# cuMF/cumf_als

Hardware: AMD Instinct MI355X
Metric: ratings/sec per ALS half-iteration (Netflix f=100); RMSE vs reference (higher is better)
Workload: dtype f32 (bf16x3-split products on the bf16 matrix pipe, fp32 accumulate); 1 GPU; netflix-shape synthetic ratings 17770x480189, nnz=99072112, f=100, lambda=0.048, solver=lu, X_BATCH=1 THETA_BATCH=1, fused Gram+solve; step=update-X + update-Theta (two half-iterations)

## Files before the change

### cumf_als_amd/als.py

```python
from __future__ import annotations

import ctypes as C

import numpy as np

from . import lib as _libmod

SOLVER_CG, SOLVER_LU = 0, 1
CUMF_ERR_FAST_RANGE = 10001


def _solver_id(solver) -> int:
    if solver in (SOLVER_CG, "cg", "CG"):
        return SOLVER_CG
    if solver in (SOLVER_LU, "lu", "LU"):
        return SOLVER_LU
    raise ValueError(f"unknown solver {solver!r}")


def _hostptr(a: np.ndarray, dtype) -> C.c_void_p:
    if a.dtype != dtype or not a.flags["C_CONTIGUOUS"]:
        raise TypeError(f"expected C-contiguous {np.dtype(dtype).name} array")
    return a.ctypes.data_as(C.c_void_p)

# ... 255 lines not shown

def lu_solve(A, b, x=None):
    import torch

    lib = _libmod.load()
    f = b.shape[-1]
    batch = b.numel() // f
    if x is None:
        x = torch.empty_like(b)
    _libmod.check(lib.cumf_lu_solve_batched(_dp(A, torch.float32), _dp(b, torch.float32), _dp(x, torch.float32),
                                            batch, f, _stream()), "cumf_lu_solve_batched")
    return x


def pack_upper(full, packed=None):
    import torch

    lib = _libmod.load()
    batch, f = full.shape[0], full.shape[-1]
    if packed is None:
        packed = torch.empty((batch, f * (f + 1) // 2), dtype=torch.float32, device=full.device)
    _libmod.check(lib.cumf_pack_upper(_dp(full, torch.float32), _dp(packed, torch.float32), batch, f, _stream()),
                  "cumf_pack_upper")
    return packed


def unpack_upper(packed, full):
    import torch

    lib = _libmod.load()
    batch, f = full.shape[0], full.shape[-1]
    _libmod.check(lib.cumf_unpack_upper(_dp(packed, torch.float32), _dp(full, torch.float32), batch, f, _stream()),
                  "cumf_unpack_upper")
    return full


def sse(val, row, col, thetaT, XT, count: int | None = None, surpass_nan: bool = False, out=None):
    import torch

    lib = _libmod.load()
    f = thetaT.shape[-1]
    if count is None:
        count = val.numel()
    if out is None:
        out = torch.zeros(1, dtype=torch.float64, device=val.device)
    _libmod.check(lib.cumf_sse(_dp(val, torch.float32), _dp(row, torch.int32), _dp(col, torch.int32),
                               _dp(thetaT, torch.float32), _dp(XT, torch.float32), int(count), f,
                               int(bool(surpass_nan)), _dp(out, torch.float64), _stream()), "cumf_sse")
    return out


GRAM_AUTO, GRAM_EXACT, GRAM_FAST = 0, 1, 2


def set_gram_mode(mode) -> None:
    m = {"auto": GRAM_AUTO, "split": GRAM_AUTO, "exact": GRAM_EXACT, "fast": GRAM_FAST}.get(mode, mode)
    _libmod.check(_libmod.load().cumf_set_gram_mode(int(m)), "cumf_set_gram_mode")


def get_gram_mode() -> str:
    return {GRAM_EXACT: "exact", GRAM_FAST: "fast"}.get(_libmod.load().cumf_get_gram_mode(), "auto")


PRESPLIT_AUTO, PRESPLIT_OFF, PRESPLIT_ON, PRESPLIT_VERIFY = -1, 0, 1, 2


def set_presplit(mode) -> None:
    m = {"auto": PRESPLIT_AUTO, "off": PRESPLIT_OFF, "on": PRESPLIT_ON, "verify": PRESPLIT_VERIFY}.get(mode, mode)
    _libmod.check(_libmod.load().cumf_set_presplit(int(m)), "cumf_set_presplit")


def get_presplit() -> str:
    return {PRESPLIT_OFF: "off", PRESPLIT_ON: "on", PRESPLIT_VERIFY: "verify"}.get(_libmod.load().cumf_get_presplit(), "auto")


def presplit_table(table: "torch.Tensor") -> "torch.Tensor":
    import torch

    lib = _libmod.load()
    rows, f = int(table.shape[0]), int(table.shape[1])
    pitch = int(lib.cumf_presplit_pitch(f))
    if pitch == 0:
        raise ValueError(f"no pre-split kernels for f = {f}")
    out = torch.empty((rows, pitch), dtype=torch.uint8, device=table.device)
    _libmod.check(lib.cumf_presplit_table(_dp(table, torch.float32), out.data_ptr(), rows, f, _stream()), "cumf_presplit_table")
    return out


def gram_fast_status() -> int:
    import ctypes as C

    flags = C.c_int(0)
    _libmod.check(_libmod.load().cumf_gram_fast_status(C.byref(flags)), "cumf_gram_fast_status")
    return int(flags.value)


def check_gram_fast() -> None:
    if _libmod.load().cumf_get_gram_mode() != GRAM_FAST:
        return
    flags = gram_fast_status()
    if flags:
        what = " and ".join(w for b, w in ((1, "a factor"), (2, "a rating")) if flags & b)
        raise RuntimeError(f"gram mode 'fast': {what} beyond the f16 range of the pre-split operands "
                           "(|value| >= 15.99): use the default gram mode")


def set_debug_switches(switches: int) -> None:
    lib = _libmod.load()
    if not hasattr(lib, "cumf_set_debug_switches"):
        raise RuntimeError("ablation switches exist only in libALS_ablate.so (load it through CUMF_ALS_LIB)")
    _libmod.check(lib.cumf_set_debug_switches(int(switches)), "cumf_set_debug_switches")


def debug_cg_histogram(f: int):
    lib = _libmod.load()
    if not hasattr(lib, "cumf_debug_cg_histogram"):
        raise RuntimeError("the CG histogram exists only in libALS_ablate.so (load it through CUMF_ALS_LIB)")
    out = (C.c_ulonglong * 16)()
    _libmod.check(lib.cumf_debug_cg_histogram(int(f), out), "cumf_debug_cg_histogram")
    return [int(v) for v in out]


def last_kernel_name() -> str:
    buf = C.create_string_buffer(256)
    _libmod.check(_libmod.load().cumf_last_kernel_name(buf, 256), "cumf_last_kernel_name")
    return buf.value.decode()


def last_tile_batches():
    info = (C.c_long * 2)()
    _libmod.check(_libmod.load().cumf_last_tile_batches(info), "cumf_last_tile_batches")
    return int(info[0]), int(info[1])


def set_kernel_timing(enable: bool) -> None:
    _libmod.check(_libmod.load().cumf_set_kernel_timing(int(bool(enable))), "cumf_set_kernel_timing")


def last_kernel_ms():
    a, b = C.c_float(), C.c_float()
    _libmod.check(_libmod.load().cumf_last_kernel_ms(C.byref(a), C.byref(b)), "cumf_last_kernel_ms")
    return a.value, b.value


def kernel_ms_since_reset():
    a, b, n = C.c_float(), C.c_float(), C.c_int()
    _libmod.check(_libmod.load().cumf_kernel_ms_since_reset(C.byref(a), C.byref(b), C.byref(n)),
                  "cumf_kernel_ms_since_reset")
    return a.value, b.value, n.value


def release_scratch() -> None:
    _libmod.check(_libmod.load().cumf_release_scratch(), "cumf_release_scratch")



NNLS_MAX_F = 128


def nnls_available(f: int) -> bool:
    return bool(_libmod.load().cumf_nnls_available(int(f)))


def _check_nonneg_f(f: int) -> None:
    if not (8 <= int(f) <= NNLS_MAX_F and int(f) % 2 == 0):
        raise ValueError(f"non-negative ALS takes even 8 <= f <= {NNLS_MAX_F} (got f = {f})")

# ... 719 lines not shown
```

### cumf_als_amd/csrc/als_capi.cpp

```cpp
#include <hip/hip_runtime.h>

#include <cxxabi.h>

#include <algorithm>
#include <cmath>
#include <cstdint>
#include <cstdio>
#include <cstdlib>
#include <cstring>
#include <vector>

#include "als_internal.h"
#include "cg.h"
#include "cumf_als_capi.h"

using namespace cumf;

namespace {

#if CUMF_ABLATE
int g_debug_switches = -1;
int debug_switches() {
  if (g_debug_switches < 0) g_debug_switches = getenv("CUMF_ALS_DBG") ? atoi(getenv("CUMF_ALS_DBG")) : 0;
  return g_debug_switches;
}
#endif

KernelArgs base_args(const cumf_plan_t* p, const int* colidx, const float* val, const float* gather, int f,
                     float lambda) {
  KernelArgs a{};
  a.item_row = p->d_item_row;
  a.item_begin = p->d_item_begin;
  a.item_len = p->d_item_len;
  a.item_slot = p->d_item_slot;
  a.item_rowlen = p->d_item_rowlen;
  a.mrow_row = p->d_mrow_row;
  a.mrow_slot0 = p->d_mrow_slot0;
  a.mrow_nslots = p->d_mrow_nslots;
  a.mrow_rowlen = p->d_mrow_rowlen;
  a.part = p->d_part;
  a.colidx = colidx;
  a.val = val;
  a.gather = gather;
  a.gather_f32 = gather;
  a.row_begin = p->row_begin;
  a.f = f;
  a.lambda = lambda;
#if CUMF_ABLATE
  a.dbg = debug_switches();
#endif
  return a;
}

int fast_words(const cumf_plan_t* p, const float* gather, int f, hipStream_t stream, KernelArgs* a) {
  if (p->gather_rows <= 0) {
    fprintf(stderr, "cumf_als_update_fused: gram mode \"fast\" needs the row count of the gather table "
                    "(cumf_plan_set_gather_rows)\n");
    return (int)hipErrorInvalidValue;
  }
  const size_t n = (size_t)p->gather_rows * f;
  void* words = nullptr;
  int rc = scratch_get(stream, kScratchWords, n * sizeof(unsigned), &words);
  if (rc) return rc;
  int* flag = nullptr;
  rc = fast_flag_get(&flag);
  if (rc) return rc;
  CUMF_HIP_CHECK(launch_presplit(gather, static_cast<unsigned*>(words), n, flag, stream));
  a->gather = reinterpret_cast<const float*>(words);
  a->fast_flag = flag;
  return 0;
}

int pre_words(const cumf_plan_t* p, const float* gather, int f, hipStream_t stream, KernelArgs* a) {
  void* planes = nullptr;
  const int rc = scratch_get(stream, kScratchPlanes, (size_t)p->gather_rows * presplit_pitch(f), &planes);
  if (rc) return rc;
  CUMF_HIP_CHECK(launch_presplit3(gather, planes, p->gather_rows, f, stream));
  a->gather = reinterpret_cast<const float*>(planes);
  a->pre_pitch = presplit_pitch(f);
  return 0;
}

thread_local int g_last_error = 0;

}


extern "C" int cumf_last_error(void) {
  const int e = g_last_error;
  g_last_error = 0;
  return e;
}
void cumf::set_last_error(int code) { g_last_error = code; }

extern "C" int cumf_last_kernel_name(char* buf, int cap) {
  if (!buf || cap <= 0) return (int)hipErrorInvalidValue;
  buf[0] = 0;
  const void* fn = last_item_kernel();
  if (!fn) return 0;
  const char* mangled = hipKernelNameRefByPtr(fn, nullptr);
  if (!mangled) return 0;
  int status = 0;
  char* dem = abi::__cxa_demangle(mangled, nullptr, nullptr, &status);
  const char* name = (status == 0 && dem) ? dem : mangled;
  size_t len = strlen(name);
  int depth = 0;
  for (size_t i = 0; name[i]; ++i) {
    if (name[i] == '<') ++depth;
    if (name[i] == '>') --depth;
    if (name[i] == '(' && depth == 0) {
      len = i;
      break;
    }
  }
  if (strncmp(name, "void ", 5) == 0) {
    name += 5;
    len -= 5;
  }
  if (len >= (size_t)cap) len = (size_t)cap - 1;
  memcpy(buf, name, len);
  buf[len] = 0;
  free(dem);
  return 0;
}

extern "C" int cumf_fused_available(int f, int solver) {
  const int mode = solver == CUMF_SOLVER_LU ? kModeLU : kModeCG;
  if (f <= 0 || (f % 2) != 0 || (solver != CUMF_SOLVER_CG && solver != CUMF_SOLVER_LU)) return 0;
  return route_for(f, mode, PlanFacts{}, switches()).path != kPathNone;
}

namespace {
int update_fused_impl(const cumf_plan_t* p, const int* colidx, const float* val, const float* gather, float* update, int f,
                      float lambda, int solver, int cg_iters, double* sse_bins, void* stream) {
  if (!p || f != p->f) {
    fprintf(stderr, "cumf_als_update_fused: plan/f mismatch\n");
    return (int)hipErrorInvalidValue;
  }
  if (!cumf_fused_available(f, solver)) {
    fprintf(stderr, "cumf_als_update_fused: f = %d with this solver needs the materialising path "
                    "(cumf_get_hermitian + cumf_*_solve_batched): the fused LU serves even f <= %d, the fused CG "
                    "too except in gram mode exact (the full system in LDS, f <= %d)\n", f, kMaxF, kVecLd);
    return (int)hipErrorInvalidValue;
  }
  ScratchLease lease;
  KernelArgs a = base_args(p, colidx, val, gather, f, lambda);
  a.update = update;
  a.cg_iters = cg_iters;
  a.sse_bins = sse_bins;
  const int mode = (solver == CUMF_SOLVER_LU) ? kModeLU : kModeCG;
  const Route r = route_for(f, mode, plan_facts(p), switches());
  PlanLists lists{};
  int rc = plan_lists(p, &lists, static_cast<hipStream_t>(stream), r.whole == kSolveTileBuffer);
  if (!rc && r.table == kTableF16Words) rc = fast_words(p, gather, f, static_cast<hipStream_t>(stream), &a);
  if (!rc && r.table == kTablePlanes) rc = pre_words(p, gather, f, static_cast<hipStream_t>(stream), &a);
  if (rc) return rc;
  CUMF_HIP_CHECK(launch_half_iteration(a, mode, r, lists, static_cast<hipStream_t>(stream)));
  return 0;
}
}

extern "C" int cumf_als_update_fused(const cumf_plan_t* p, const int* colidx, const float* val, const float* gather,
// ... 272 lines not shown
```

### cumf_als_amd/csrc/als_dual.hip

```cpp
#include <hip/hip_runtime.h>

#include "als_device.h"
#include "als_internal.h"
#include "als_lu_blocked.h"
#include "als_wave_gram.h"
#include "als_wave_solve.h"

namespace cumf {

namespace {

constexpr int kDualFB = 6;
constexpr int kDualPlane = 32 * kDualFB;
constexpr int kDualChunks = kDualFB / 2;
constexpr int kDualStrip = 96 * kDualFB;
constexpr int kDualWaves = 3;
constexpr int kDualPass = 40;

template <class T>
__device__ __forceinline__ __attribute__((address_space(1))) const T* as_global(const void* p) {
  return reinterpret_cast<__attribute__((address_space(1))) const T*>(reinterpret_cast<unsigned long long>(p));
}

template <int NBD>
__host__ __device__ constexpr int dual_lds_floats() {
  return wave_lu_lds_floats<NBD>(16 * NBD - 1) + 16 * NBD + 16;
}

template <int NBD, int KC>
__device__ __forceinline__ void dual_load_chunk(const char* const (&ptr)[NBD], u32x4 (&op)[NBD][3]) {
  static_for<NBD>([&](auto ic) {
    constexpr int I = decltype(ic)::value;
    static_for<3>([&](auto pc) {
      constexpr int p = decltype(pc)::value;
      op[I][p] = *as_global<u32x4>(ptr[I] + kDualPlane * p + 64 * KC);
    });
  });
}
template <int NBD>
__device__ __forceinline__ void dual_products(const u32x4 (&op)[NBD][3], f32x4 (&acc)[NBD * (NBD + 1) / 2]) {
  static_for<6>([&](auto prc) {
    constexpr int PROD = decltype(prc)::value;
    constexpr int pa = PROD == 0 ? 2 : (PROD == 2 || PROD == 3) ? 1 : 0;
    constexpr int pb = PROD == 1 ? 2 : (PROD == 2 || PROD == 4) ? 1 : 0;
    static_for<NBD*(NBD + 1) / 2>([&](auto tc) {
      constexpr int t = decltype(tc)::value;
      constexpr int I = tile_I<NBD>(t), J = tile_J<NBD>(t);
      acc[t] = mfma_bf16(op[I][pa], op[J][pb], acc[t]);
    });
  });
}

template <int NBD>
__global__ __launch_bounds__(64, kDualWaves) void als_dual_kernel(const KernelArgs a) {
  extern __shared__ __attribute__((aligned(16))) float smem[];
  constexpr int NT = NBD * (NBD + 1) / 2;
  constexpr int kMaxN = 16 * NBD - 1;
  const int lane = threadIdx.x;
  const int item = blockIdx.x;
  const int row = a.item_row[item];
  const long long begin = a.item_begin[item];
  const int n = a.item_len[item];
  const int f = a.f;
  const int c = lane & 15, g = lane >> 4;
  auto bperm_i = [](int addr, int v) { return __builtin_amdgcn_ds_bpermute(addr, v); };

  const bool l0 = lane < n, l1 = 64 + lane < n;
  const int i0 = l0 ? a.colidx[begin + lane] : 0, i1 = l1 ? a.colidx[begin + 64 + lane] : 0;
  const float r0 = (l0 && a.val != nullptr) ? a.val[begin + lane] : 0.f;
  const float r1 = (l1 && a.val != nullptr) ? a.val[begin + 64 + lane] : 0.f;

  const char* ptr[NBD];
  static_for<NBD>([&](auto ic) {
    constexpr int I = decltype(ic)::value;
    const int idx = bperm_i(4 * ((16 * I + c) & 63), 16 * I < 64 ? i0 : i1);
    const char* p = reinterpret_cast<const char*>(a.gather) + (unsigned long long)(unsigned)idx * a.pre_pitch;
    ptr[I] = (16 * I + c < n ? p : reinterpret_cast<const char*>(g_wave_zeros)) + 16 * g;
  });

  f32x4 acc[NT];
#pragma unroll
  for (int t = 0; t < NT; ++t) acc[t] = f32x4{0.f, 0.f, 0.f, 0.f};

  static_for<kDualChunks>([&](auto kcc) {
    u32x4 op[NBD][3];
    dual_load_chunk<NBD, decltype(kcc)::value>(ptr, op);
    dual_products<NBD>(op, acc);
  });
  if ((f & 15) != 0) {
    const bool g0 = g == 0, g1 = g == 1, g2 = g == 2, g03 = g == 0 || g == 3;
    u32x4 A[NBD], B[NBD];
    static_for<NBD>([&](auto ic) {
      constexpr int I = decltype(ic)::value;
      const char* sp = ptr[I] + (kDualStrip - 16 * g);
      const u32x2 h = *as_global<u32x2>(sp), m = *as_global<u32x2>(sp + 8), l = *as_global<u32x2>(sp + 16);
      const u32x2 alo = (g0 || g1) ? h : (g2 ? m : l), ahi = g0 ? h : ((g1 || g2) ? m : l);
      const u32x2 blo = g03 ? h : (g1 ? l : m), bhi = g03 ? m : (g1 ? h : l);
      A[I] = u32x4{alo[0], alo[1], ahi[0], ahi[1]};
      B[I] = u32x4{blo[0], blo[1], bhi[0], bhi[1]};
    });
    static_for<NT>([&](auto tc) {
      constexpr int t = decltype(tc)::value;
      constexpr int I = tile_I<NBD>(t), J = tile_J<NBD>(t);
      acc[t] = mfma_bf16(A[I], B[J], acc[t]);
    });
  }

  const int np = n > 16 * (NBD - 1) ? n : 16 * (NBD - 1);
  const int cr = np - 16 * (NBD - 1);
  static_for<NBD>([&](auto ic) {
    constexpr int I = decltype(ic)::value;
    constexpr int t = tile_of<NBD>(I, NBD - 1);
#pragma unroll
    for (int r = 0; r < 4; ++r) {
      const int rho = 16 * I + 4 * g + r;
      const float v = __builtin_bit_cast(float, bperm_i(4 * (rho & 63), __builtin_bit_cast(int, 16 * I < 64 ? r0 : r1)));
      acc[t][r] = c == cr ? v : acc[t][r];
    }
  });

  const float reg = (float)n * a.lambda;
  float* ybuf = smem + wave_lu_lds_floats<NBD>(kMaxN);
  if (lane < 32) ybuf[16 * (NBD - 1) + lane] = 0.f;
  const float ssq = lu_wave_blocked<NBD, 0>(acc, smem, np, reg, ybuf, lane);
  __syncthreads();
  if (a.sse_bins != nullptr) {
    const float yy = wave_sum_uniform(ssq);
    wave_sse_add(a.sse_bins, (double)reg * (double)reg * (double)yy, n, lane);
  }

  const int off1 = 64 + lane < f ? 64 + lane : lane;
  float x0 = 0.f, x1 = 0.f;
  static_for<(kMaxN + kDualPass) / kDualPass>([&](auto pc) {
    constexpr int r0p = kDualPass * decltype(pc)::value;
    if (r0p < n) {
      float T0[kDualPass], T1[kDualPass];
      static_for<kDualPass / 8>([&](auto qc) {
        constexpr int q = decltype(qc)::value;
        if (r0p + 8 * q < n) {
          static_for<8>([&](auto ec) {
            constexpr int e = 8 * q + decltype(ec)::value, rho = r0p + e;
            const int rc = rho < n ? rho : n - 1;
            const int idx = __builtin_amdgcn_readlane(rho < 64 ? i0 : i1, rc & 63);
            const auto base = as_global<float>(a.gather_f32 + (size_t)(unsigned)idx * f);
            T0[e] = base[lane];
            T1[e] = base[off1];
          });
        }
      });
      static_for<kDualPass / 8>([&](auto qc) {
        constexpr int q = decltype(qc)::value;
        if (r0p + 8 * q < n) {
          static_for<8>([&](auto ec) {
            constexpr int e = 8 * q + decltype(ec)::value, rho = r0p + e;
            const float y = ybuf[rho];
            x0 = fmaf(T0[e], y, x0);
            x1 = fmaf(T1[e], y, x1);
          });
        }
      });
    }
  });
  const bool f0 = lane < f, f1 = 64 + lane < f;
  float* xg = a.update + (size_t)row * f;
  if (f0) xg[lane] = x0;
  if (f1) xg[64 + lane] = x1;
}

}

bool dual_rows_available(int f) { return nb_for_f(f) == 7 && presplit_supported(f); }

hipError_t launch_dual_rows(const KernelArgs& a, long n_items, hipStream_t stream) {
  if (n_items <= 0) return hipSuccess;
  if (!dual_rows_available(a.f) || a.gather_f32 == nullptr || a.pre_pitch != presplit_pitch(a.f)) return hipErrorInvalidValue;
  static_assert(kDualMaxRow == 16 * 5 - 1, "NBD = 5");
  return launch_kernel(als_dual_kernel<5>, dim3((unsigned)n_items), dim3(64), dual_lds_floats<5>() * sizeof(float), stream, a);
// ... 4 lines not shown
```

### cumf_als_amd/csrc/als_internal.h

```cpp
#ifndef CUMF_ALS_INTERNAL_H_
#define CUMF_ALS_INTERNAL_H_

#include <hip/hip_runtime.h>

#include <algorithm>
#include <cstddef>
#include <type_traits>

#ifndef CUMF_ABLATE
#define CUMF_ABLATE 0
#endif

namespace cumf {

constexpr int kThreads = 256;
constexpr int kStage = 32;
constexpr int kVecLd = 128;
constexpr int kMaxFusedNB = 9;
constexpr int kMaxF = 207;
constexpr int kMaxFAny = 512;
constexpr int kMaxWaveNB = 7;
constexpr int kMaxFusedLuWaveNB = 9;

enum { kModeCG = 0, kModeLU = 1, kModeMaterialize = 2, kModeLUExact = 3, kModeCGHalf = 4 };

__host__ __device__ constexpr int nb_for_f(int f) { return f / 16 + 1; }
constexpr int kMaxNB = nb_for_f(kMaxF);
__host__ __device__ constexpr int solve_ldg(int f, int mode) { return mode == kModeCG ? ((f + 1 + 3) & ~3) : (f + 1); }
__host__ __device__ constexpr size_t solve_g_floats(int f, int mode) {
  return ((size_t)f * solve_ldg(f, mode) + 3) & ~(size_t)3;
}
__host__ __device__ constexpr size_t lu_packed_floats(int nb) { return (size_t)256 * nb * (nb + 1) / 2 + 16 * nb; }
__host__ __device__ constexpr size_t lu_lds_floats(int nb, int f) { return lu_packed_floats(nb) + (size_t)((f + 3) & ~3) + 48; }
constexpr int kCgExtraFloats = 12 * kVecLd;
__host__ __device__ constexpr size_t solve_lds_floats(int f, int mode) {
  return solve_g_floats(f, mode) + (mode == kModeCG ? (size_t)kCgExtraFloats : 0);
}

__host__ __device__ constexpr bool fused_supported(int f, int mode) {
  return mode == kModeLU ? nb_for_f(f) <= nb_for_f(kMaxF) : (f <= kVecLd && nb_for_f(f) <= kMaxFusedNB);
}

struct KernelArgs {
  const int* item_row;
  const long long* item_begin;
  const int* item_len;
  const int* item_slot;
  const int* item_rowlen;
  const int* mrow_row;
  const int* mrow_slot0;
  const int* mrow_nslots;
  const int* mrow_rowlen;
  float* part;
  const int* colidx;
  const float* val;
  const float* gather;
  float* update;
  float* tt;
  float* rhs;
  int tt_half;
  int tt_packed;
  int dense_slots;
  int whole_only;
  long long row_begin;
  int f;
  float lambda;
  int cg_iters;
  int dbg;
  int fast_words;
  int* fast_flag;
  int pre_words;
  unsigned pre_pitch;
  double* sse_bins;
  const float* gather_f32;
  int no_pack;
};
constexpr int kSseBins = 1024;

struct PlanLists {
  long n_items, n_mrows;
  long n_citems, n_witems;
  const int *c_row, *c_len, *c_slot, *c_rowlen;
  const long long* c_begin;
  const int *w_row, *w_len, *w_rowlen;
  const long long* w_begin;
  float* part2;
  long part2_rows;
  double chunk_share;
  long n_short;
};
constexpr int kShortRow = 32;
bool short_cg_available(int f);
hipError_t launch_short_cg(const KernelArgs& a, long n_items, hipStream_t stream);
constexpr int kDualMaxRow = 79, kDualMaxRow6 = 95;
bool dual_rows_available(int f);
hipError_t launch_dual_rows(const KernelArgs& a, long n_items, hipStream_t stream);
hipError_t launch_solve_batched(const float* A, const float* b, float* x, long batch, int f, int mode, int cg_iters,
                                hipStream_t stream);
enum { kGramAuto = 0, kGramExact = 1, kGramFast = 2 };
enum { kArithSplit3 = 0, kArithFast = 1, kArithPre = 2, kArithPrePk = 3, kArithSplitPk = 4 };

struct Switches {
  int gram;
  int presplit;
  double presplit_mb;
  bool splitpk;
  bool short_cg;
  bool dual;
  bool batched;
  bool wave_solve;
  bool lu_exact;
};
Switches switches();
void set_gram_mode(int mode);
void set_presplit_mode(int mode);

struct PlanFacts {
  int nb;
  long n_mrows, n_citems, n_witems;
  double chunk_share;
  long n_short;
  long gather_rows;
  long n_dual;
  long n_empty;
};
enum Path {
  kPathNone,
  kPathGeneric,
  kPathWorkgroup,
  kPathOneWave,
  kPathTwoWave,
};
enum Table { kTableNone, kTablePlanes, kTableF16Words };
enum Solve {
  kSolveInKernel,
  kSolveTileBuffer,
  kSolveReduce,
  kSolveWaveCG,
};
struct Route {
  Path path;
  int arith;
  int fc;
  Table table;
  bool chunk_first;
  long n_short;
  Solve chunked;
  Solve whole;
  bool sse;
  long n_dual, n_dual_behind;
};
Route route_for(int f, int mode, const PlanFacts& plan, const Switches& sw);
hipError_t launch_half_iteration(const KernelArgs& a, int mode, const Route& r, const PlanLists& lists, hipStream_t stream);

hipError_t launch_presplit(const float* src, unsigned* dst, size_t n, int* flag, hipStream_t stream);
hipError_t launch_gram_generic(const KernelArgs& a, long n_items, hipStream_t stream);
hipError_t launch_lu_global(const float* A, float* work, const float* b, float* x, long batch, int f, hipStream_t stream);
__host__ __device__ constexpr bool presplit_supported(int f) {
  return ((nb_for_f(f) == 7 || nb_for_f(f) == 5) && ((f & 15) == 0 || (f & 15) == 4)) ||
         (nb_for_f(f) > kMaxWaveNB && nb_for_f(f) <= nb_for_f(kMaxF) && (f & 3) == 0 && (f & 15) <= 8);
}
__host__ __device__ constexpr bool presplit_pays(int f) { return presplit_supported(f) && nb_for_f(f) >= 7; }
__host__ __device__ constexpr bool presplit_pays_any_size(int f) { return presplit_supported(f) && nb_for_f(f) >= 10; }
__host__ __device__ constexpr unsigned presplit_pitch(int f) {
  return 96u * (f / 16) + ((f & 15) ? (nb_for_f(f) > kMaxWaveNB ? 64u : 32u) : 0u);
}
hipError_t launch_presplit3(const float* src, void* dst, long long rows, int f, hipStream_t stream);
hipError_t launch_pack_upper(const float* full, float* packed, long batch, int f, int unpack, hipStream_t stream);
void set_last_error(int code);
void set_kernel_timing(bool on);
void note_item_kernel(const void* host_function);
const void* last_item_kernel();
hipError_t last_kernel_ms(float* item_ms, float* reduce_ms);
hipError_t kernel_ms_since_reset(float* item_ms, float* reduce_ms, int* launches);
hipError_t launch_quadratic_terms(const float* A, const float* b, const float* x, const float* reg, long batch, int f,
                                  double* out, hipStream_t stream);
hipError_t launch_sse(const float* val, const int* row, const int* col, const float* thetaT, const float* XT,
                      long count, int f, int surpass_nan, double* out, hipStream_t stream);
hipError_t launch_cg_global(const float* A, const float* b, float* x, long batch, int f, int cg_iters, bool a_half,
                            hipStream_t stream);

template <int NB>
hipError_t slice_half_iteration(const KernelArgs& a, int mode, long n_items, long n_mrows, hipStream_t stream);
template <int NB>
hipError_t slice_solve(const float* A, const float* b, float* x, long batch, int f, int mode, int cg_iters,
                       hipStream_t stream);
template <int NB>
hipError_t slice_reduce_only(const KernelArgs& a, int mode, const Route& r, long n_mrows, hipStream_t stream);
template <int NB>
hipError_t wave_item_launch(const KernelArgs& a, int mode, const Route& r, bool whole, long n_items, hipStream_t stream);
template <int NB>
hipError_t wave_solve_launch(const KernelArgs& a, int mode, long n_rows, hipStream_t stream);
template <int NB>
hipError_t wave_lu_launch(const KernelArgs& a, const Route& r, bool whole, long n_items, hipStream_t stream);
template <int NB>
hipError_t wave_cg_hist(unsigned long long* out16);

template <int LO, int HI, class Go>
hipError_t with_nb(int nb, Go&& go) {
  if constexpr (LO > HI)
    return hipErrorInvalidValue;
  else
    return nb == LO ? go(std::integral_constant<int, LO>{}) : with_nb<LO + 1, HI>(nb, go);
}

#define CUMF_LOCAL __attribute__((visibility("hidden")))

enum {
  kScratchTiles = 0,
  kScratchWords = 1,
  kScratchPlanes = 2,
  kScratchImpGram = 3,
  kScratchImpSlots = 4,
  kScratchImpTT = 5,
  kScratchImpRhs = 6,
  kScratchImpX = 7,
  kScratchImpAux = 8,
  kScratchTopkWork = 9,
  kScratchTopkPart = 10,
  kScratchTopkMetrics = 11,
  kScratchNnlsTT = 12,
  kScratchNnlsRhs = 13,
  kScratchRankKeys = 14,
  kScratchRankHist = 15,
  kScratchRankValid = 16,
  kScratchRankMetrics = 17,
  kScratchLuWork = 18,
  kScratchBiasResid = 19,
  kScratchBiasPart = 20,
  kScratchFreeVec = 21,
  kScratchFreePart = 22,
  kScratchFreeWords = 23,
};
int scratch_get(hipStream_t stream, int kind, size_t bytes, void** out);
template <typename T>
CUMF_LOCAL inline int scratch(hipStream_t stream, int kind, size_t count, T** out) {
  void* q = nullptr;
  const int rc = scratch_get(stream, kind, (count ? count : 1) * sizeof(T), &q);
  *out = static_cast<T*>(q);
  return rc;
}
CUMF_LOCAL size_t scratch_capacity(hipStream_t stream, int kind);
CUMF_LOCAL int fast_flag_get(int** out);
struct ScratchLease {
  int dev = 0;
  ScratchLease();
  ~ScratchLease();
  ScratchLease(const ScratchLease&) = delete;
// ... 75 lines not shown
```

### cumf_als_amd/csrc/als_route.cpp

```cpp
#include <cstdlib>

#include "als_internal.h"
#include "cumf_als_capi.h"

namespace cumf {

namespace {
int g_gram_mode = -1;
int g_presplit_mode = -2;
}

void set_gram_mode(int mode) { g_gram_mode = (mode == kGramExact || mode == kGramFast) ? mode : kGramAuto; }
void set_presplit_mode(int mode) { g_presplit_mode = mode; }

Switches switches() {
  if (g_gram_mode < 0) {
    const char* e = getenv("CUMF_ALS_GRAM");
    g_gram_mode = (e && (e[0] == 'e' || e[0] == 'E')) ? kGramExact : (e && (e[0] == 'f' || e[0] == 'F')) ? kGramFast : kGramAuto;
  }
  if (g_presplit_mode == -2) {
    const char* e = getenv("CUMF_ALS_PRESPLIT");
    g_presplit_mode = (e && e[0] == '0') ? CUMF_PRESPLIT_OFF : (e && e[0] == '1') ? CUMF_PRESPLIT_ON
                      : (e && e[0] == '2') ? CUMF_PRESPLIT_VERIFY : CUMF_PRESPLIT_AUTO;
  }
  static const double presplit_mb = getenv("CUMF_ALS_PRESPLIT_MB") ? atof(getenv("CUMF_ALS_PRESPLIT_MB")) : 64.0;
  static const bool splitpk = !(getenv("CUMF_ALS_SPLITPK") && *getenv("CUMF_ALS_SPLITPK") == '0');
  static const bool short_cg = !getenv("CUMF_ALS_SHORT_CG") || atoi(getenv("CUMF_ALS_SHORT_CG")) != 0;
  const char* dual = getenv("CUMF_ALS_DUAL");
  const char* lu_exact = getenv("CUMF_ALS_LU_EXACT");
  return Switches{g_gram_mode,
                  g_presplit_mode,
                  presplit_mb,
                  splitpk,
                  short_cg,
                  !dual || atoi(dual) != 0,
                  !getenv("CUMF_ALS_NO_BATCHED"),
                  !getenv("CUMF_ALS_NO_WAVE_SOLVE"),
                  lu_exact && atoi(lu_exact) != 0};
}

static bool presplit_wanted(int f, long gather_rows, const Switches& sw) {
  if (sw.presplit == CUMF_PRESPLIT_OFF || sw.gram != kGramAuto || !presplit_supported(f) || gather_rows <= 0) return false;
  if (sw.presplit == CUMF_PRESPLIT_ON || sw.presplit == CUMF_PRESPLIT_VERIFY) return true;
  return presplit_pays_any_size(f) || (presplit_pays(f) && (double)gather_rows * presplit_pitch(f) <= sw.presplit_mb * 1048576.0);
}

Route route_for(int f, int mode, const PlanFacts& p, const Switches& sw) {
  Route r{};
  const int nb = nb_for_f(f);
  const bool wave_gram = sw.gram != kGramExact;
  if (f > kMaxF)
    r.path = mode == kModeMaterialize ? kPathGeneric : kPathNone;
  else if (wave_gram && nb >= 2 && nb <= kMaxWaveNB)
    r.path = kPathOneWave;
  else if (wave_gram && sw.batched && nb > kMaxWaveNB)
    r.path = kPathTwoWave;
  else
    r.path = (mode == kModeMaterialize || fused_supported(f, mode)) ? kPathWorkgroup : kPathNone;
  const bool one = r.path == kPathOneWave, wave = one || r.path == kPathTwoWave;

  r.arith = kArithSplit3;
  if (wave && mode != kModeMaterialize) {
    if (sw.gram == kGramFast) {
      r.table = kTableF16Words;
      r.arith = kArithFast;
    } else if (presplit_wanted(f, p.gather_rows, sw)) {
      r.table = kTablePlanes;
      r.arith = (one && sw.presplit != CUMF_PRESPLIT_VERIFY) ? kArithPrePk : kArithPre;
    } else if (one && sw.splitpk && (f & 15) == 0 && sw.presplit != CUMF_PRESPLIT_OFF &&
               sw.presplit != CUMF_PRESPLIT_VERIFY) {
      r.arith = kArithSplitPk;
    }
  }
  r.fc = (one && f == 100) ? 100 : 0;

  r.chunked = (wave && mode == kModeCG && sw.wave_solve && (one || f > kVecLd)) ? kSolveWaveCG : kSolveReduce;
  r.whole = (r.path == kPathTwoWave && mode != kModeCG && !(mode == kModeLU && nb <= kMaxFusedLuWaveNB)) ? kSolveTileBuffer
                                                                                                          : kSolveInKernel;
  r.chunk_first = one && mode == kModeLU && p.n_mrows > 0 && p.n_citems > 0 && p.n_witems > 0 && p.chunk_share < 0.25;
  r.n_short = (one && mode == kModeCG && sw.short_cg && short_cg_available(f)) ? p.n_short : 0;
  const bool dual = one && mode == kModeLU && sw.dual && r.arith == kArithPrePk && nb == 7 && (f & 3) == 0 && f >= 96 &&
                    dual_rows_available(f);
  r.n_dual = dual ? p.n_dual : 0;
  r.n_dual_behind = r.n_dual > 0 ? p.n_empty : 0;
  r.sse = wave && mode != kModeMaterialize &&
          (p.n_mrows == 0 || r.chunked == kSolveWaveCG || (mode == kModeLU && nb >= 7));
  return r;
}

}
```

### cumf_als_amd/csrc/als_wave.hip

```cpp
#include <hip/hip_runtime.h>

#include <cstdio>
#include <cstdlib>
#include <type_traits>

#ifndef CUMF_WAVE_NB
#error "compile with -DCUMF_WAVE_NB=<feature blocks>"
#endif

#include "als_device.h"
#include "als_lu_wg.h"
#include "als_lu_blocked.h"
#include "als_internal.h"
#include "als_wave_gram.h"
#include "als_wave_pre.h"
#include "als_wave_solve.h"

namespace cumf {

#define CUMF_WAVE_PRE (CUMF_WAVE_NB == 7 || CUMF_WAVE_NB == 5)
#define CUMF_WAVE_SPLITPK (CUMF_WAVE_NB <= 7)

template <int NB, int NW>
__global__ __launch_bounds__(64 * NW, 2) void als_wave_cg_kernel(const KernelArgs a) {
// ... 350 lines not shown
#endif
#if CUMF_WAVE_PRE
    case kArithPrePk: return at(std::integral_constant<int, kArithPrePk>{});
#endif
#if CUMF_WAVE_SPLITPK
    case kArithSplitPk: return at(std::integral_constant<int, kArithSplitPk>{});
#endif
    default: return hipErrorInvalidValue;
  }
}

#if CUMF_WAVE_PART == 1 && CUMF_WAVE_NB <= 7
template <int NB, int FC, int ARITH, bool WHOLE>
static hipError_t launch_wave_lu_w(const KernelArgs& a, long n_items, hipStream_t stream) {
  const size_t stage_lds = wave_stage_lds_floats<NB, ARITH>() * sizeof(float);
  const size_t lu_lds = wave_lu_lds_floats<NB>(a.f) * sizeof(float);
  const size_t lds = lu_lds > stage_lds ? lu_lds : stage_lds;
  if (n_items <= 0) {
    note_item_kernel(reinterpret_cast<const void*>(als_wave_kernel<NB, kModeLU, FC, ARITH, WHOLE>));
    return hipSuccess;
  }
  return launch_item_kernel(als_wave_kernel<NB, kModeLU, FC, ARITH, WHOLE>, dim3((unsigned)n_items), dim3(64), lds, stream, a);
}
template <int NB>
hipError_t wave_lu_launch(const KernelArgs& a, const Route& r, bool whole, long n_items, hipStream_t stream) {
  return with_arith(r, [&](auto arith, auto fc) {
    constexpr int ARITH = decltype(arith)::value, FC = decltype(fc)::value;
    return whole ? launch_wave_lu_w<NB, FC, ARITH, true>(a, n_items, stream)
                 : launch_wave_lu_w<NB, FC, ARITH, false>(a, n_items, stream);
  });
}
#endif

#if CUMF_WAVE_PART == 0
template <int NB, int FC, int ARITH>
static hipError_t launch_wave_fc(const KernelArgs& a, int mode, long n_items, hipStream_t stream) {
  const size_t stage_lds = wave_stage_lds_floats<NB, ARITH>() * sizeof(float);
  if (mode != kModeMaterialize)
    return launch_item_kernel(als_wave_kernel<NB, kModeCG, FC, ARITH>, dim3((unsigned)n_items), dim3(64), stage_lds, stream, a);
  if constexpr (ARITH != kArithSplit3) {
    return hipErrorInvalidValue;
  } else {
    return launch_item_kernel(als_wave_kernel<NB, kModeMaterialize, FC, kArithSplit3>, dim3((unsigned)n_items), dim3(64),
                              stage_lds, stream, a);
  }
}

template <int NB>
hipError_t wave_item_launch(const KernelArgs& a, int mode, const Route& r, bool whole, long n_items, hipStream_t stream) {
  if (n_items <= 0 && !(mode == kModeLU && NB <= kMaxWaveNB && r.n_dual > 0)) return hipSuccess;
  if (mode != kModeMaterialize && mode != kModeLU && mode != kModeCG) return hipErrorInvalidValue;
  if constexpr (NB > kMaxWaveNB) {
    return with_arith(r, [&](auto arith, auto) -> hipError_t {
      constexpr int ARITH = decltype(arith)::value;
      if (ARITH != kArithSplit3 && mode == kModeMaterialize) return hipErrorInvalidValue;
      size_t lds = ARITH == kArithPre ? PreGeo2<NB>::kBytes : 2 * wave_stage_lds_floats<NB>() * sizeof(float);
      if (lu_wg_lds_floats<NB>(a.f) * sizeof(float) > lds) lds = lu_wg_lds_floats<NB>(a.f) * sizeof(float);
      const auto kernel = mode == kModeCG ? als_wave_multi_kernel<NB, 2, kModeCG, ARITH>
                                          : als_wave_multi_kernel<NB, 2, kModeLU, ARITH>;
      return launch_item_kernel(kernel, dim3((unsigned)n_items), dim3(128), lds, stream, a);
    });
  } else {
    if (mode == kModeLU) return wave_lu_launch<NB>(a, r, whole, n_items, stream);
    return with_arith(r, [&](auto arith, auto fc) {
      return launch_wave_fc<NB, decltype(fc)::value, decltype(arith)::value>(a, mode, n_items, stream);
    });
  }
}

#endif

#if CUMF_ABLATE && CUMF_WAVE_PART == 0
template <int NB>
hipError_t wave_cg_hist(unsigned long long* out16) {
  hipError_t e = hipMemcpyFromSymbol(out16, HIP_SYMBOL(g_cg_hist), 16 * sizeof(unsigned long long));
  if (e != hipSuccess) return e;
  const unsigned long long zero[16] = {};
  return hipMemcpyToSymbol(HIP_SYMBOL(g_cg_hist), zero, sizeof(zero));
}
#endif

#if CUMF_WAVE_PART == 0 && CUMF_WAVE_NB == 7
__global__ __launch_bounds__(256) void presplit_bf16x3_kernel(const float* __restrict__ src, unsigned short* __restrict__ dst,
                                                              long long n, int f, int fb, int sw, unsigned pitch_halfs) {
  const long long i = (long long)blockIdx.x * 256 + threadIdx.x;
  if (i >= n) return;
  const long long row = i / f;
  const int k = (int)(i - row * f);
  unsigned H, M, L;
  split3_pair(src[i], 0.f, H, M, L);
  unsigned short* r = dst + row * pitch_halfs;
  if (k < 16 * fb) {
    r[k] = (unsigned short)H;
    r[16 * fb + k] = (unsigned short)M;
    r[32 * fb + k] = (unsigned short)L;
  } else {
    const int e = k - 16 * fb, sf = f - 16 * fb;
    unsigned short* st = r + 48 * fb;
    st[e] = (unsigned short)H;
    st[sw + e] = (unsigned short)M;
    st[2 * sw + e] = (unsigned short)L;
    if (e == 0) {
      for (int p = 0; p < 3; ++p)
        for (int z = sf; z < sw; ++z) st[p * sw + z] = 0;
      for (int z = 0; z < sw; ++z) st[3 * sw + z] = 0;
    }
  }
}
hipError_t launch_presplit3(const float* src, void* dst, long long rows, int f, hipStream_t stream) {
  const long long n = rows * f;
  if (n <= 0) return hipSuccess;
  if (!presplit_supported(f)) return hipErrorInvalidValue;
  const int fb = f / 16;
  const unsigned pitch = presplit_pitch(f);
  return launch_kernel(presplit_bf16x3_kernel, dim3((unsigned)((n + 255) / 256)), dim3(256), 0, stream, src,
                       static_cast<unsigned short*>(dst), n, f, fb, nb_for_f(f) > kMaxWaveNB ? 8 : 4, pitch / 2);
}
#endif

#if CUMF_WAVE_PART == 0
template hipError_t wave_item_launch<CUMF_WAVE_NB>(const KernelArgs&, int, const Route&, bool, long, hipStream_t);
template hipError_t wave_solve_launch<CUMF_WAVE_NB>(const KernelArgs&, int, long, hipStream_t);
#if CUMF_ABLATE
template hipError_t wave_cg_hist<CUMF_WAVE_NB>(unsigned long long*);
#endif
#elif CUMF_WAVE_NB <= 7
template hipError_t wave_lu_launch<CUMF_WAVE_NB>(const KernelArgs&, const Route&, bool, long, hipStream_t);
#endif

}
```

### cumf_als_amd/csrc/als_wave_pre.h

```cpp
#pragma once
#include "als_wave_gram.h"

namespace cumf {

typedef short s16x4 __attribute__((ext_vector_type(4)));
typedef __attribute__((address_space(3))) s16x4* lds_tr_ptr;
typedef char __attribute__((address_space(3)))* lds_byte_ptr;
template <int NB>
struct PreGeo {
  static constexpr int FB = NB - 1;
  static constexpr int RP = FB <= 2 ? 64 : 192;
  static constexpr int LP = RP / 16;
  static constexpr int CS = 4 * RP;
  static constexpr int kMain = 24 * CS + 3 * 32;
  static constexpr int kStrip = kMain;
  static constexpr int kZero = kStrip + 1024;
  static constexpr int kRating = kZero + 32;
  __host__ __device__ static constexpr int bytes(bool packed) { return packed ? kRating : kRating + 768; }
  static_assert(32 * FB <= RP && 4 * LP <= 64, "a rating's plane fits its slot, four ratings fit the wave");
  __host__ __device__ static constexpr int chunk(int E, int p) { return (3 * E + p) * CS + 32 * (E >> 1); }
};

template <int NB>
struct PreStage {
  int idx[8];
  int sidx;
  float rv;
};
template <int NB, bool PK>
struct PreGather {
  using G = PreGeo<NB>;
  const char* lane_base;
  const char* zero_base;
  const char* strip_base;
  const char* strip_zero;
  const int* ib;
  const float* vb;
  lds_tr_ptr tr_main;
  lds_tr_ptr tr_last[2];
  unsigned pitch;
  int len, q, lane;
#if CUMF_ABLATE_STAGE
  int dbg;
#endif
  bool dma_active, sp;

  __device__ __forceinline__ void init(const KernelArgs& a, int f, long long begin, int len_, int lane_, float* smem) {
    lane = lane_;
    len = len_;
    pitch = a.pre_pitch;
#if CUMF_ABLATE
    if (a.dbg & 8) pitch = 0u;
#endif
#if CUMF_ABLATE_STAGE
    dbg = a.dbg;
#endif
    sp = ((f & 15) >> 2) != 0;
    q = lane / G::LP;
    const int piece = lane % G::LP;
    dma_active = q < 4 && piece < 2 * G::FB;
    q = q < 4 ? q : 3;
    lane_base = reinterpret_cast<const char*>(a.gather) + 16 * piece;
    zero_base = reinterpret_cast<const char*>(g_wave_zeros) + 16 * piece;
    strip_base = reinterpret_cast<const char*>(a.gather) + 96 * G::FB + 16 * (lane & 1);
    strip_zero = reinterpret_cast<const char*>(g_wave_zeros) + 16 * (lane & 1);
    ib = len_ > 0 ? a.colidx + begin : reinterpret_cast<const int*>(g_wave_zeros);
    vb = (len_ > 0 && a.val != nullptr) ? a.val + begin : g_wave_zeros;
    const int g = lane >> 4, j = (lane >> 2) & 3, aa = lane & 3;
    lds_byte_ptr base = (lds_byte_ptr)smem;
    tr_main = (lds_tr_ptr)(base + 6 * g * G::CS + 32 * g + G::RP * j + 8 * aa);
    const int spn = sp ? 1 : 0;
#pragma unroll
    for (int u = 0; u < 2; ++u) {
      const int rho = 8 * g + 4 * u + j;
      int off;
      if constexpr (PK)
        off = (sp || aa == 0) ? G::kStrip + 32 * rho + (sp ? 8 * aa : 24) : G::kZero;
      else
        off = aa < spn ? G::kStrip + 32 * rho + 8 * aa : (aa == spn ? G::kRating + 24 * rho : G::kZero);
      tr_last[u] = (lds_tr_ptr)(base + off);
    }
    constexpr int kClear = (G::bytes(PK) - G::kZero) / 16;
    if (lane < kClear) reinterpret_cast<f32x4*>(reinterpret_cast<char*>(smem) + G::kZero)[lane] = f32x4{0.f, 0.f, 0.f, 0.f};
  }

  template <bool FULL>
  __device__ __forceinline__ void load_idx(PreStage<NB>& st, int s) const {
    const int top = len > 0 ? len - 1 : 0;
    if constexpr (FULL) {
      const int* p = ib + kWaveStage * s + q;
#pragma unroll
      for (int E = 0; E < 8; ++E) st.idx[E] = p[4 * E];
      st.sidx = ib[kWaveStage * s + (lane >> 1)];
    } else {
#pragma unroll
      for (int E = 0; E < 8; ++E) {
        const int pos = kWaveStage * s + 4 * E + q;
        st.idx[E] = ib[pos < top ? pos : top];
      }
      const int ps = kWaveStage * s + (lane >> 1);
      st.sidx = ib[ps < top ? ps : top];
    }
  }
  template <bool FULL>
  __device__ __forceinline__ void load_rv(PreStage<NB>& st, int s) const {
    const int pv = kWaveStage * s + (lane & 31);
    if constexpr (FULL) {
      st.rv = vb[pv];
    } else {
      const int top = len > 0 ? len - 1 : 0;
      const float v = vb[pv < top ? pv : top];
      st.rv = pv < len ? v : 0.f;
    }
  }

  __device__ __forceinline__ void put_rating(const PreStage<NB>& st, float* smem) const {
    unsigned H, M, L;
    split3_pair(st.rv, 0.f, H, M, L);
    if (lane < 32) {
      if constexpr (PK) {
        u32x2 w = {(H & 0xffffu) | (M << 16), L & 0xffffu};
        *reinterpret_cast<u32x2*>(reinterpret_cast<char*>(smem) + G::kStrip + 32 * lane + 24) = w;
      } else {
        unsigned short* rp = reinterpret_cast<unsigned short*>(reinterpret_cast<char*>(smem) + G::kRating + 24 * lane);
        rp[0] = (unsigned short)H;
        rp[4] = (unsigned short)M;
        rp[8] = (unsigned short)L;
      }
    }
  }

  template <bool FULL>
  __device__ __forceinline__ void dma_issue(const PreStage<NB>& st, float* smem, int s) const {
#if defined(__HIP_DEVICE_COMPILE__)
    using gptr = const __attribute__((address_space(1))) void*;
    using lptr = __attribute__((address_space(3))) void*;
    lds_byte_ptr lds = (lds_byte_ptr)smem;
    if (dma_active) {
      static_for<8>([&](auto ec) {
        constexpr int E = decltype(ec)::value;
        const char* row = lane_base + (unsigned long long)(unsigned)st.idx[E] * pitch;
        if constexpr (!FULL) row = (kWaveStage * s + 4 * E + q < len) ? row : zero_base;
        static_for<3>([&](auto pc) {
          constexpr int p = decltype(pc)::value;
          __builtin_amdgcn_global_load_lds((gptr)row, (lptr)(lds + G::chunk(E, p) - 32 * G::FB * p), 16, 32 * G::FB * p, 0);
        });
      });
    }
    if (sp) {
      const char* row = strip_base + (unsigned long long)(unsigned)st.sidx * pitch;
      if constexpr (!FULL) row = (kWaveStage * s + (lane >> 1) < len) ? row : strip_zero;
      __builtin_amdgcn_global_load_lds((gptr)row, (lptr)(lds + G::kStrip), 16, 0, 0);
    }
#endif
  }

  static __device__ __forceinline__ u32x2 tr_read(lds_tr_ptr p, int byte_off) {
    return __builtin_bit_cast(u32x2, __builtin_amdgcn_ds_read_tr16_b64_v4i16((lds_tr_ptr)((lds_byte_ptr)p + byte_off)));
  }
  template <int B0, int B1, class PL>
  __device__ __forceinline__ void read_blocks(PL& P) const {
    static_for<B1 - B0>([&](auto bc) {
      constexpr int B = B0 + decltype(bc)::value;
      static_for<2>([&](auto uc) {
        constexpr int u = decltype(uc)::value;
        const u32x2 vh = tr_read(tr_main, (3 * u + 0) * G::CS + 32 * B);
        const u32x2 vm = tr_read(tr_main, (3 * u + 1) * G::CS + 32 * B);
        const u32x2 vl = tr_read(tr_main, (3 * u + 2) * G::CS + 32 * B);
        P.h[B][2 * u] = vh[0], P.h[B][2 * u + 1] = vh[1];
        P.m[B][2 * u] = vm[0], P.m[B][2 * u + 1] = vm[1];
        P.l[B][2 * u] = vl[0], P.l[B][2 * u + 1] = vl[1];
      });
    });
  }
  template <class PL>
  __device__ __forceinline__ void read_pk(PL& P) const {
    const u32x2 v0 = tr_read(tr_last[0], 0), v1 = tr_read(tr_last[1], 0);
    P.pk = u32x4{v0[0], v0[1], v1[0], v1[1]};
  }
  template <class PL>
  __device__ __forceinline__ void read(PL& P) const {
    if constexpr (PK) read_pk(P);
    static_for<G::FB>([&](auto bc) {
      constexpr int B = decltype(bc)::value;
      static_for<2>([&](auto uc) {
        constexpr int u = decltype(uc)::value;
        const u32x2 vh = tr_read(tr_main, (3 * u + 0) * G::CS + 32 * B);
        const u32x2 vm = tr_read(tr_main, (3 * u + 1) * G::CS + 32 * B);
        const u32x2 vl = tr_read(tr_main, (3 * u + 2) * G::CS + 32 * B);
        P.h[B][2 * u] = vh[0], P.h[B][2 * u + 1] = vh[1];
        P.m[B][2 * u] = vm[0], P.m[B][2 * u + 1] = vm[1];
        P.l[B][2 * u] = vl[0], P.l[B][2 * u + 1] = vl[1];
      });
    });
    if constexpr (!PK) {
      constexpr int B = G::FB;
      const u32x2 h0 = tr_read(tr_last[0], 0), m0 = tr_read(tr_last[0], 8), l0 = tr_read(tr_last[0], 16);
      const u32x2 h1 = tr_read(tr_last[1], 0), m1 = tr_read(tr_last[1], 8), l1 = tr_read(tr_last[1], 16);
      P.h[B] = u32x4{h0[0], h0[1], h1[0], h1[1]};
      P.m[B] = u32x4{m0[0], m0[1], m1[0], m1[1]};
      P.l[B] = u32x4{l0[0], l0[1], l1[0], l1[1]};
    }
  }
};

template <int NB, int KIND, bool PK, class PL>
__device__ __forceinline__ void stage_step_pre(const PreGather<NB, PK>& wg, PL& P, PreStage<NB>& R, float* smem,
                                               f32x4 (&acc)[NB * (NB + 1) / 2], int s_next, int s_load) {
  __builtin_amdgcn_s_waitcnt(0x0F70);
  wg.put_rating(R, smem);
  wg.read(P);
  __builtin_amdgcn_s_waitcnt(0xC07F);
  if constexpr (KIND == kStepFull) {
    wg.template dma_issue<true>(R, smem, s_next);
    wg.template load_idx<true>(R, s_load);
    wg.template load_rv<true>(R, s_next);
  } else if constexpr (KIND == kStepPartial) {
    const int nfull = wg.len / kWaveStage, nst = (wg.len + kWaveStage - 1) / kWaveStage;
    if (s_next < nfull) {
      wg.template dma_issue<true>(R, smem, s_next);
      wg.template load_rv<true>(R, s_next);
    } else {
      wg.template dma_issue<false>(R, smem, s_next);
      wg.template load_rv<false>(R, s_next);
    }
    if (s_load < nfull)
      wg.template load_idx<true>(R, s_load);
    else if (s_load < nst)
      wg.template load_idx<false>(R, s_load);
  }
  u32x4 h2[2] = {{0u, 0u, 0u, 0u}, {0u, 0u, 0u, 0u}};
  static_for<GramSched<NB>::N>([&](auto nc) { gram_mfma_sched<NB, GramSched, decltype(nc)::value>(P, acc, h2); });
}

// ... 193 lines not shown
```

Baseline: 11.93 billion ratings/s.

## Use 32-bit offsets and an in-table zero row for pre-split gathers

Replaces 64-bit per-row pointers into the pre-split bf16x3 table with 32-bit byte offsets computed via __umul24, and routes out-of-range rows to an appended zero row inside the table instead of a separate global zero buffer. It also pads the pitch to a 128-byte multiple for the wave path and zero-fills the padding. The aim is to cut address-computation VGPRs and instructions in the gather and DMA paths and to improve alignment of row loads. In exchange the table grows by one row plus padding, and tables too large for 32-bit offsets or 24-bit row indices fall back to a non-pre-split route.

```diff
diff --git a/cumf_als_amd/als.py b/cumf_als_amd/als.py
--- a/cumf_als_amd/als.py
+++ b/cumf_als_amd/als.py
@@ -361,7 +361,7 @@
     pitch = int(lib.cumf_presplit_pitch(f))
     if pitch == 0:
         raise ValueError(f"no pre-split kernels for f = {f}")
-    out = torch.empty((rows, pitch), dtype=torch.uint8, device=table.device)
+    out = torch.empty((rows + 1, pitch), dtype=torch.uint8, device=table.device)
     _libmod.check(lib.cumf_presplit_table(_dp(table, torch.float32), out.data_ptr(), rows, f, _stream()), "cumf_presplit_table")
     return out
 
diff --git a/cumf_als_amd/csrc/als_capi.cpp b/cumf_als_amd/csrc/als_capi.cpp
--- a/cumf_als_amd/csrc/als_capi.cpp
+++ b/cumf_als_amd/csrc/als_capi.cpp
@@ -73,11 +73,12 @@
 
 int pre_words(const cumf_plan_t* p, const float* gather, int f, hipStream_t stream, KernelArgs* a) {
   void* planes = nullptr;
-  const int rc = scratch_get(stream, kScratchPlanes, (size_t)p->gather_rows * presplit_pitch(f), &planes);
+  const int rc = scratch_get(stream, kScratchPlanes, (size_t)presplit_table_bytes(p->gather_rows, f), &planes);
   if (rc) return rc;
   CUMF_HIP_CHECK(launch_presplit3(gather, planes, p->gather_rows, f, stream));
   a->gather = reinterpret_cast<const float*>(planes);
   a->pre_pitch = presplit_pitch(f);
+  a->pre_zero_row = (unsigned)p->gather_rows;
   return 0;
 }
 
diff --git a/cumf_als_amd/csrc/als_dual.hip b/cumf_als_amd/csrc/als_dual.hip
--- a/cumf_als_amd/csrc/als_dual.hip
+++ b/cumf_als_amd/csrc/als_dual.hip
@@ -28,12 +28,12 @@
 }
 
 template <int NBD, int KC>
-__device__ __forceinline__ void dual_load_chunk(const char* const (&ptr)[NBD], u32x4 (&op)[NBD][3]) {
+__device__ __forceinline__ void dual_load_chunk(const char* table, const unsigned (&off)[NBD], u32x4 (&op)[NBD][3]) {
   static_for<NBD>([&](auto ic) {
     constexpr int I = decltype(ic)::value;
     static_for<3>([&](auto pc) {
       constexpr int p = decltype(pc)::value;
-      op[I][p] = *as_global<u32x4>(ptr[I] + kDualPlane * p + 64 * KC);
+      op[I][p] = *as_global<u32x4>(table + off[I] + (kDualPlane * p + 64 * KC));
     });
   });
 }
@@ -70,12 +70,12 @@
   const float r0 = (l0 && a.val != nullptr) ? a.val[begin + lane] : 0.f;
   const float r1 = (l1 && a.val != nullptr) ? a.val[begin + 64 + lane] : 0.f;
 
-  const char* ptr[NBD];
+  const char* table = reinterpret_cast<const char*>(a.gather);
+  unsigned off[NBD];
   static_for<NBD>([&](auto ic) {
     constexpr int I = decltype(ic)::value;
-    const int idx = bperm_i(4 * ((16 * I + c) & 63), 16 * I < 64 ? i0 : i1);
-    const char* p = reinterpret_cast<const char*>(a.gather) + (unsigned long long)(unsigned)idx * a.pre_pitch;
-    ptr[I] = (16 * I + c < n ? p : reinterpret_cast<const char*>(g_wave_zeros)) + 16 * g;
+    const unsigned idx = (unsigned)bperm_i(4 * ((16 * I + c) & 63), 16 * I < 64 ? i0 : i1);
+    off[I] = __umul24(16 * I + c < n ? idx : a.pre_zero_row, a.pre_pitch) + 16u * (unsigned)g;
   });
 
   f32x4 acc[NT];
@@ -84,7 +84,7 @@
 
   static_for<kDualChunks>([&](auto kcc) {
     u32x4 op[NBD][3];
-    dual_load_chunk<NBD, decltype(kcc)::value>(ptr, op);
+    dual_load_chunk<NBD, decltype(kcc)::value>(table, off, op);
     dual_products<NBD>(op, acc);
   });
   if ((f & 15) != 0) {
@@ -92,7 +92,7 @@
     u32x4 A[NBD], B[NBD];
     static_for<NBD>([&](auto ic) {
       constexpr int I = decltype(ic)::value;
-      const char* sp = ptr[I] + (kDualStrip - 16 * g);
+      const char* sp = table + (off[I] - 16u * (unsigned)g) + kDualStrip;
       const u32x2 h = *as_global<u32x2>(sp), m = *as_global<u32x2>(sp + 8), l = *as_global<u32x2>(sp + 16);
       const u32x2 alo = (g0 || g1) ? h : (g2 ? m : l), ahi = g0 ? h : ((g1 || g2) ? m : l);
       const u32x2 blo = g03 ? h : (g1 ? l : m), bhi = g03 ? m : (g1 ? h : l);
diff --git a/cumf_als_amd/csrc/als_internal.h b/cumf_als_amd/csrc/als_internal.h
--- a/cumf_als_amd/csrc/als_internal.h
+++ b/cumf_als_amd/csrc/als_internal.h
@@ -69,7 +69,7 @@
   int dbg;
   int fast_words;
   int* fast_flag;
-  int pre_words;
+  unsigned pre_zero_row;
   unsigned pre_pitch;
   double* sse_bins;
   const float* gather_f32;
@@ -162,8 +162,19 @@
 }
 __host__ __device__ constexpr bool presplit_pays(int f) { return presplit_supported(f) && nb_for_f(f) >= 7; }
 __host__ __device__ constexpr bool presplit_pays_any_size(int f) { return presplit_supported(f) && nb_for_f(f) >= 10; }
+__host__ __device__ constexpr unsigned presplit_payload(int f) {
+  return 96u * (f / 16) + ((f & 15) ? (nb_for_f(f) > kMaxWaveNB ? 64u : 32u) : 0u);
+}
 __host__ __device__ constexpr unsigned presplit_pitch(int f) {
-  return 96u * (f / 16) + ((f & 15) ? (nb_for_f(f) > kMaxWaveNB ? 64u : 32u) : 0u);
+  return nb_for_f(f) > kMaxWaveNB ? presplit_payload(f) : (presplit_payload(f) + 127u) / 128u * 128u;
+}
+constexpr long kPlanesMaxRows = 1L << 24;
+constexpr unsigned long long kPlanesMaxBytes = 1ULL << 32;
+__host__ __device__ constexpr unsigned long long presplit_table_bytes(long rows, int f) {
+  return (unsigned long long)(rows + 1) * presplit_pitch(f);
+}
+__host__ __device__ constexpr bool presplit_offsets_fit(long rows, int f) {
+  return rows < kPlanesMaxRows && presplit_table_bytes(rows, f) < kPlanesMaxBytes;
 }
 hipError_t launch_presplit3(const float* src, void* dst, long long rows, int f, hipStream_t stream);
 hipError_t launch_pack_upper(const float* full, float* packed, long batch, int f, int unpack, hipStream_t stream);
diff --git a/cumf_als_amd/csrc/als_route.cpp b/cumf_als_amd/csrc/als_route.cpp
--- a/cumf_als_amd/csrc/als_route.cpp
+++ b/cumf_als_amd/csrc/als_route.cpp
@@ -42,7 +42,7 @@
 static bool presplit_wanted(int f, long gather_rows, const Switches& sw) {
   if (sw.presplit == CUMF_PRESPLIT_OFF || sw.gram != kGramAuto || !presplit_supported(f) || gather_rows <= 0) return false;
   if (sw.presplit == CUMF_PRESPLIT_ON || sw.presplit == CUMF_PRESPLIT_VERIFY) return true;
-  return presplit_pays_any_size(f) || (presplit_pays(f) && (double)gather_rows * presplit_pitch(f) <= sw.presplit_mb * 1048576.0);
+  return presplit_pays_any_size(f) || (presplit_pays(f) && (double)gather_rows * presplit_payload(f) <= sw.presplit_mb * 1048576.0);
 }
 
 Route route_for(int f, int mode, const PlanFacts& p, const Switches& sw) {
@@ -65,8 +65,10 @@
       r.table = kTableF16Words;
       r.arith = kArithFast;
     } else if (presplit_wanted(f, p.gather_rows, sw)) {
-      r.table = kTablePlanes;
-      r.arith = (one && sw.presplit != CUMF_PRESPLIT_VERIFY) ? kArithPrePk : kArithPre;
+      if (!one || presplit_offsets_fit(p.gather_rows, f)) {
+        r.table = kTablePlanes;
+        r.arith = (one && sw.presplit != CUMF_PRESPLIT_VERIFY) ? kArithPrePk : kArithPre;
+      }
     } else if (one && sw.splitpk && (f & 15) == 0 && sw.presplit != CUMF_PRESPLIT_OFF &&
                sw.presplit != CUMF_PRESPLIT_VERIFY) {
       r.arith = kArithSplitPk;
diff --git a/cumf_als_amd/csrc/als_wave.hip b/cumf_als_amd/csrc/als_wave.hip
--- a/cumf_als_amd/csrc/als_wave.hip
+++ b/cumf_als_amd/csrc/als_wave.hip
@@ -456,14 +456,21 @@
 
 #if CUMF_WAVE_PART == 0 && CUMF_WAVE_NB == 7
 __global__ __launch_bounds__(256) void presplit_bf16x3_kernel(const float* __restrict__ src, unsigned short* __restrict__ dst,
-                                                              long long n, int f, int fb, int sw, unsigned pitch_halfs) {
+                                                              long long n, long long rows, int f, int fb, int sw,
+                                                              unsigned pitch_halfs, unsigned pay_halfs) {
   const long long i = (long long)blockIdx.x * 256 + threadIdx.x;
-  if (i >= n) return;
+  if (i >= n) {
+    const long long j = i - n;
+    if (j < pitch_halfs / 8) reinterpret_cast<u32x4*>(dst + rows * pitch_halfs)[j] = u32x4{0u, 0u, 0u, 0u};
+    return;
+  }
   const long long row = i / f;
   const int k = (int)(i - row * f);
   unsigned H, M, L;
   split3_pair(src[i], 0.f, H, M, L);
   unsigned short* r = dst + row * pitch_halfs;
+  if (k == 0)
+    for (unsigned z = pay_halfs; z < pitch_halfs; z += 8) *reinterpret_cast<u32x4*>(r + z) = u32x4{0u, 0u, 0u, 0u};
   if (k < 16 * fb) {
     r[k] = (unsigned short)H;
     r[16 * fb + k] = (unsigned short)M;
@@ -483,12 +490,13 @@
 }
 hipError_t launch_presplit3(const float* src, void* dst, long long rows, int f, hipStream_t stream) {
   const long long n = rows * f;
-  if (n <= 0) return hipSuccess;
-  if (!presplit_supported(f)) return hipErrorInvalidValue;
+  if (rows < 0 || !presplit_supported(f)) return hipErrorInvalidValue;
   const int fb = f / 16;
   const unsigned pitch = presplit_pitch(f);
-  return launch_kernel(presplit_bf16x3_kernel, dim3((unsigned)((n + 255) / 256)), dim3(256), 0, stream, src,
-                       static_cast<unsigned short*>(dst), n, f, fb, nb_for_f(f) > kMaxWaveNB ? 8 : 4, pitch / 2);
+  const long long threads = n + pitch / 16;
+  return launch_kernel(presplit_bf16x3_kernel, dim3((unsigned)((threads + 255) / 256)), dim3(256), 0, stream, src,
+                       static_cast<unsigned short*>(dst), n, rows, f, fb, nb_for_f(f) > kMaxWaveNB ? 8 : 4, pitch / 2,
+                       presplit_payload(f) / 2);
 }
 #endif
 
diff --git a/cumf_als_amd/csrc/als_wave_pre.h b/cumf_als_amd/csrc/als_wave_pre.h
--- a/cumf_als_amd/csrc/als_wave_pre.h
+++ b/cumf_als_amd/csrc/als_wave_pre.h
@@ -30,10 +30,10 @@
 template <int NB, bool PK>
 struct PreGather {
   using G = PreGeo<NB>;
-  const char* lane_base;
-  const char* zero_base;
-  const char* strip_base;
-  const char* strip_zero;
+  const char* table;
+  unsigned lane_off;
+  unsigned strip_off;
+  unsigned zero_row;
   const int* ib;
   const float* vb;
   lds_tr_ptr tr_main;
@@ -60,10 +60,10 @@
     const int piece = lane % G::LP;
     dma_active = q < 4 && piece < 2 * G::FB;
     q = q < 4 ? q : 3;
-    lane_base = reinterpret_cast<const char*>(a.gather) + 16 * piece;
-    zero_base = reinterpret_cast<const char*>(g_wave_zeros) + 16 * piece;
-    strip_base = reinterpret_cast<const char*>(a.gather) + 96 * G::FB + 16 * (lane & 1);
-    strip_zero = reinterpret_cast<const char*>(g_wave_zeros) + 16 * (lane & 1);
+    table = reinterpret_cast<const char*>(a.gather);
+    lane_off = 16u * (unsigned)piece;
+    strip_off = 96u * G::FB + 16u * (unsigned)(lane & 1);
+    zero_row = a.pre_zero_row;
     ib = len_ > 0 ? a.colidx + begin : reinterpret_cast<const int*>(g_wave_zeros);
     vb = (len_ > 0 && a.val != nullptr) ? a.val + begin : g_wave_zeros;
     const int g = lane >> 4, j = (lane >> 2) & 3, aa = lane & 3;
@@ -139,8 +139,9 @@
     if (dma_active) {
       static_for<8>([&](auto ec) {
         constexpr int E = decltype(ec)::value;
-        const char* row = lane_base + (unsigned long long)(unsigned)st.idx[E] * pitch;
-        if constexpr (!FULL) row = (kWaveStage * s + 4 * E + q < len) ? row : zero_base;
+        unsigned idx = (unsigned)st.idx[E];
+        if constexpr (!FULL) idx = (kWaveStage * s + 4 * E + q < len) ? idx : zero_row;
+        const char* row = table + (__umul24(idx, pitch) + lane_off);
         static_for<3>([&](auto pc) {
           constexpr int p = decltype(pc)::value;
           __builtin_amdgcn_global_load_lds((gptr)row, (lptr)(lds + G::chunk(E, p) - 32 * G::FB * p), 16, 32 * G::FB * p, 0);
@@ -148,8 +149,9 @@
       });
     }
     if (sp) {
-      const char* row = strip_base + (unsigned long long)(unsigned)st.sidx * pitch;
-      if constexpr (!FULL) row = (kWaveStage * s + (lane >> 1) < len) ? row : strip_zero;
+      unsigned idx = (unsigned)st.sidx;
+      if constexpr (!FULL) idx = (kWaveStage * s + (lane >> 1) < len) ? idx : zero_row;
+      const char* row = table + (__umul24(idx, pitch) + strip_off);
       __builtin_amdgcn_global_load_lds((gptr)row, (lptr)(lds + G::kStrip), 16, 0, 0);
     }
 #endif
```

Result: faster. 12.18 billion ratings/s, median of 6 (+2.1%).
